# LemonATsu/UNet-PhaseGen

Hardware: AMD Instinct MI355X
Metric: spectrogram-frames/sec (train fwd+bwd) (higher is better)
Workload: dtype f32; 1 GPU; train.py full step (fwd + cos/sin/mag loss + bwd + Adam), UNetModel(1024, 2048), per-GPU batch 64 x 1024 bins x 256 frames (BASELINE configs[2]); global_batch=64, frames=256, channels=1024, parallelism=dp1, grad_allreduce_payload=fp32, adam=fused into the wgrad epilogues

## Files before the change

### unet-phasegen_amd/csrc/conv_raw_wgrad.hip

```cpp
#include "conv_common.h"

namespace {

template <int KW, int S> struct GRaw {
    static constexpr int WL = 15 * S + KW;
    static constexpr int WLP = g_wlp(KW, S);
    static constexpr int NQT = RBN / KW;
    static constexpr int TNV = NQT * KW;
    static constexpr int SUB = NQT * WLP;
    static constexpr int SUBS = (SUB + 63) / 64 * 64;
    static constexpr int NE = (SUB + NT - 1) / NT;
    static constexpr int STG = RTILE_A + 2 * SUBS;
    static constexpr int SUBP = (SUB + 255) / 256 * 256;
    static_assert(WL <= WLP, "window does not fit its slot");
};

template <int KW, int S, int BF>
__device__ __forceinline__ void g_raw_bf(const IgemmParams& p) {
    using C = GRaw<KW, S>;
    __shared__ __attribute__((aligned(16))) float lds[2 * C::STG];
    const int tid = threadIdx.x, lane = tid & 63;
    const int wv = __builtin_amdgcn_readfirstlane(tid >> 6), wm = wv >> 1, wn = wv & 1;
    const int kt = dma_kt(lane, wv);
    const rsrc_t rp = make_rsrc(p.pt, p.pt_bytes), rx = make_rsrc(p.x, p.x_bytes);
    const float slopeA = act_slope(p.act_p), slopeB = act_slope(p.act_x);
    const int pbs4 = (int)p.pt_bs * 4, xbs4 = (int)p.x_bs * 4;
    const int g = logical_wg(blockIdx.x, gridDim.x, p.whole);
    const Split sp = make_split(p.tilesM * p.tilesN, p.nslab, gridDim.x, p.whole);
    int pos = split_lo(sp, g);
    const int pos_end = split_lo(sp, g + 1);
    int slot = 0;
    while (pos < pos_end) {
        const int tile = pos / p.nslab, sb = pos - tile * p.nslab;
        const int se = min(p.nslab, sb + (pos_end - pos));
        const int m0 = (tile / p.tilesN) * RBM, n0 = (tile % p.tilesN) * C::TNV;
        const int qbase = (tile % p.tilesN) * C::NQT;

        int aoff[8];
#pragma unroll
        for (int e = 0; e < 8; ++e) {
            const int m = m0 + dma_row(lane, wv, e);
            aoff[e] = m < p.M ? m * p.LP * 4 : FAR;
        }
        constexpr bool RECOMP = KW <= 5 && BF != 0;
        int choff[RECOMP ? 1 : C::NE], vv[RECOMP ? 1 : C::NE];
        if (!RECOMP) {
#pragma unroll
            for (int e = 0; e < C::NE; ++e) {
                const int idx = tid + NT * e, ql = idx / C::WLP, v = idx - ql * C::WLP;
                choff[e] = (idx < C::SUB && qbase + ql < p.Q) ? (qbase + ql) * p.Lx * 4 : FAR;
                vv[e] = v - p.p;
            }
        }
#define GRAW_CHOFF(e) (RECOMP ? ({ int t_ = tid; asm volatile("" : "+v"(t_)); const int idx_ = t_ + NT * (e), ql_ = idx_ / C::WLP; \
                                  (idx_ < C::SUB && qbase + ql_ < p.Q) ? (qbase + ql_) * p.Lx * 4 : FAR; }) : choff[RECOMP ? 0 : (e)])
#define GRAW_VV(e) (RECOMP ? ({ int t_ = tid; asm volatile("" : "+v"(t_)); const int idx_ = t_ + NT * (e); idx_ - (idx_ / C::WLP) * C::WLP - p.p; }) \
                           : vv[RECOMP ? 0 : (e)])
        constexpr bool FASTP = BF != 2 && !(KW <= 5 && BF != 0);
        constexpr bool FASTW = FASTP && KW != 4;
        constexpr int NE16 = (C::SUB / 4 + NT - 1) / NT;
        static_assert(C::WLP % 4 == 0, "16-byte window pieces");
        int pv[FASTP ? 2 : 1], woff[FASTW ? NE16 : 1];
        if (FASTW) {
#pragma unroll
            for (int e = 0; e < NE16; ++e) {
                const int f = 4 * (tid + NT * e), ql = f / C::WLP, v0 = f - ql * C::WLP;
                woff[e] = (f < C::SUB && qbase + ql < p.Q) ? ((qbase + ql) * p.Lx + v0) * 4 : FAR;
            }
        }
        if (FASTP) {
#pragma unroll
            for (int e = 0; e < 2; ++e) {
                const int m = m0 + dma16_row(lane, wv, e);
                pv[e] = m < p.M ? (m * p.LP + dma16_kc(lane)) * 4 : FAR;
            }
        }
        int bbase[4];
#pragma unroll
        for (int jb = 0; jb < 4; ++jb) {
            const int c = wn * 128 + jb * 32 + (lane & 31), qc = c / KW;
            bbase[jb] = qc * C::WLP + (c - qc * KW) + S * 8 * (lane >> 5);
        }
        AccR acc;
#pragma unroll
        for (int i = 0; i < 2; ++i)
#pragma unroll
            for (int j = 0; j < 4; ++j)
#pragma unroll
                for (int r = 0; r < 16; ++r) acc.c[i][j][r] = 0.f;

        int gb, gi;
        { const int k0 = sb * BK; gb = k0 / p.LP; gi = k0 - gb * p.LP; }
        int kc_cur = 16;

#define GRAW_ISSUE(STAGE_PTR, K0)                                                                         \
    {   float* const As = (STAGE_PTR) + wv * 64; float* const Bw = (STAGE_PTR) + RTILE_A + wv * 64;       \
        const int k0 = (K0);                                                                              \
        const int kc = p.LP - gi;                            \
        if (FASTP && kc >= 16 && gb < p.B) {                                                              \
            const int sa = gb * pbs4 + gi * 4;                                                            \
            _Pragma("unroll") for (int e = 0; e < 2; ++e) dma16s(rp, As + wv * 192 + e * 1024, pv[FASTP ? e : 0], sa); \
        } else {                                                                                          \
          int bb, ii; divmod24(k0 + kt, p.LP, p.inv_LP, bb, ii);                                          \
          const int po = bb < p.B ? bb * pbs4 + ii * 4 : OOB;                                             \
          _Pragma("unroll") for (int e = 0; e < 8; ++e) dma4(rp, As + e * 256, aoff[e] + po); }           \
        const int w0 = S * gi - p.p;                             \
        if (FASTW && kc >= 16 && gb < p.B && w0 >= 0 && w0 + C::WLP <= p.Lx) {    \
            const int sw_ = gb * xbs4 + w0 * 4;                                                           \
            _Pragma("unroll") for (int e = 0; e < NE16; ++e)                                              \
                if (4 * (e * NT + wv * 64) < C::SUB) dma16s(rx, (STAGE_PTR) + RTILE_A + 4 * (e * NT + wv * 64), woff[FASTW ? e : 0], sw_); \
        } else {                                                                                          \
        const int sb0 = gb < p.B ? gb * xbs4 : -NEVER, sb1 = (kc < 16 && gb + 1 < p.B) ? (gb + 1) * xbs4 : -NEVER; \
        _Pragma("unroll") for (int e = 0; e < C::NE; ++e) {                                               \
            if ((e + 1) * NT <= C::SUB || e * NT + wv * 64 < C::SUB) {                                    \
                const int ps = S * gi + GRAW_VV(e);                                                       \
                dma4(rx, Bw + e * NT, ((unsigned)ps < (unsigned)p.Lx && sb0 >= 0) ? sb0 + GRAW_CHOFF(e) + ps * 4 : FAR); \
            }                                                                                             \
        }                                                                                                 \
        if (kc < 16) {                                  \
            _Pragma("unroll") for (int e = 0; e < C::NE; ++e) {                                           \
                if ((e + 1) * NT <= C::SUB || e * NT + wv * 64 < C::SUB) {                                                          \
                    const int ps = GRAW_VV(e);                                                            \
                    dma4(rx, Bw + C::SUBS + e * NT, ((unsigned)ps < (unsigned)p.Lx && sb1 >= 0) ? sb1 + GRAW_CHOFF(e) + ps * 4 : FAR); \
                }                                                                                         \
            }                                                                                             \
        }                                                                                                 \
        }                                                                                                 \
        kc_next = kc < 16 ? kc : 16;                                                                      \
        gi += BK; if (gi >= p.LP) { gi -= p.LP; ++gb; }                                                   \
    }

        PG_STAMP_DECL
        int kc_next;
        GRAW_ISSUE(lds, sb * BK)
        kc_cur = kc_next;
        __syncthreads();
        for (int sl = sb; sl < se; ++sl) {
            const int cur = (sl - sb) & 1;
            PG_STAMP(0)
#if defined(PG_G_ABL) && PG_G_ABL == 1
            kc_next = 16;
#else
            GRAW_ISSUE(lds + (cur ^ 1) * C::STG, (sl + 1) * BK)
#endif
            __builtin_amdgcn_sched_barrier(0);
            PG_STAMP(1)
            {
                const float* As = lds + cur * C::STG;
                const float* Bw = As + RTILE_A;
                const int r = lane & 31, h = lane >> 5, sw = (r >> 2) & 3;
                const float* ap = As + (wm * 64 + r) * BK;
                f32x4 a[2][2];
                float b[4][8];
                if (kc_cur >= 16) {
#pragma unroll
                    for (int i = 0; i < 2; ++i) a[i][0] = *reinterpret_cast<const f32x4*>(ap + i * 32 * BK + (((2 * h) ^ sw) << 2));
#pragma unroll
                    for (int ip = 0; ip < 4; ++ip) {
                        if (ip == 2) {
#pragma unroll
                            for (int i = 0; i < 2; ++i) a[i][1] = *reinterpret_cast<const f32x4*>(ap + i * 32 * BK + (((2 * h + 1) ^ sw) << 2));
                        }
#pragma unroll
                        for (int jb = 0; jb < 4; ++jb) { b[jb][2 * ip] = Bw[bbase[jb] + S * 2 * ip]; b[jb][2 * ip + 1] = Bw[bbase[jb] + S * (2 * ip + 1)]; }
                    }
                } else {
#pragma unroll
                    for (int c = 0; c < 2; ++c)
#pragma unroll
                        for (int i = 0; i < 2; ++i) a[i][c] = *reinterpret_cast<const f32x4*>(ap + i * 32 * BK + (((2 * h + c) ^ sw) << 2));
                    typedef const volatile __attribute__((address_space(3))) float* lds_vptr;
                    const lds_vptr Bv = (lds_vptr)Bw;
                    const int shift = C::SUBS - S * kc_cur;
#pragma unroll
                    for (int i = 0; i < 8; ++i) {
                        const int d = (8 * h + i >= kc_cur) ? shift : 0;
#pragma unroll
                        for (int jb = 0; jb < 4; ++jb) b[jb][i] = Bv[bbase[jb] + S * i + d];
                    }
                }
                if (slopeA != 1.0f) {
#pragma unroll
                    for (int i = 0; i < 2; ++i)
#pragma unroll
                        for (int c = 0; c < 2; ++c)
#pragma unroll
                            for (int v = 0; v < 4; ++v) a[i][c][v] = act_apply(a[i][c][v], slopeA);
                }
                if (slopeB != 1.0f) {
#pragma unroll
                    for (int jb = 0; jb < 4; ++jb)
#pragma unroll
                        for (int i = 0; i < 8; ++i) b[jb][i] = act_apply(b[jb][i], slopeB);
                }
                if (BF) mfma_low_2x4<BF>(a, b, acc);
                else {
#pragma unroll
                    for (int kk = 0; kk < 8; ++kk) {
#pragma unroll
                        for (int i = 0; i < 2; ++i)
#pragma unroll
                            for (int j = 0; j < 4; ++j)
                                acc.c[i][j] = __builtin_amdgcn_mfma_f32_32x32x2f32(a[i][kk >> 2][kk & 3], b[j][kk], acc.c[i][j], 0, 0, 0);
                    }
                }
            }
            __builtin_amdgcn_sched_barrier(0);
            PG_STAMP(2)
            kc_cur = kc_next;
#if defined(PG_G_ABL) && PG_G_ABL == 2
            asm volatile("s_waitcnt lgkmcnt(0)\n\ts_barrier" ::: "memory");
#else
            __syncthreads();
#endif
            PG_STAMP(3)
        }
        PG_STAMP_FLUSH
#undef GRAW_ISSUE
#undef GRAW_CHOFF
#undef GRAW_VV
        if (sb == 0 && se == p.nslab) epilogue_g<S, 2, 4>(p, acc, m0, n0, lane, wm, wn, n0 + C::TNV);
        else store_partial(p.ws, g, slot, acc, tid);
        pos += se - sb;
        slot = 1;
    }
}

template <int KW, int S, int BF>
__device__ __forceinline__ void g_ps_bf(const IgemmParams& p) {
    using C = GRaw<KW, S>;
    constexpr int STG = RTILE_A + (C::SUB + 255) / 256 * 256;
    constexpr int NE16 = (C::SUB / 4 + NT - 1) / NT;
    static_assert(C::WLP % 4 == 0 && C::WLP <= 64, "16-byte window pieces; channel 0 inside the first 64 floats");
    __shared__ __attribute__((aligned(16))) float lds[2 * STG];
    const int tid = threadIdx.x, lane = tid & 63;
    const int wv = __builtin_amdgcn_readfirstlane(tid >> 6), wm = wv >> 1, wn = wv & 1;
    const rsrc_t rp = make_rsrc(p.pt, p.pt_bytes), rx = make_rsrc(p.x, p.x_bytes);
    const float slopeA = act_slope(p.act_p), slopeB = act_slope(p.act_x);
    const int pbs4 = (int)p.pt_bs * 4, xbs4 = (int)p.x_bs * 4;
    const int cps = (p.LP + 15) >> 4;
    const int g = logical_wg(blockIdx.x, gridDim.x, p.whole);
    const Split sp = make_split(p.tilesM * p.tilesN, p.nslab, gridDim.x, p.whole);
    int pos = split_lo(sp, g);
    const int pos_end = split_lo(sp, g + 1);
    int slot = 0;
    while (pos < pos_end) {
        const int tile = pos / p.nslab, sb = pos - tile * p.nslab;
        const int se = min(p.nslab, sb + (pos_end - pos));
        const int m0 = (tile / p.tilesN) * RBM, n0 = (tile % p.tilesN) * C::TNV;
        const int qbase = (tile % p.tilesN) * C::NQT;

        int pv[2], woff[NE16];
#pragma unroll
        for (int e = 0; e < 2; ++e) {
            const int m = m0 + dma16_row(lane, wv, e);
            pv[e] = m < p.M ? (m * p.LP + dma16_kc(lane)) * 4 : FAR;
        }
#pragma unroll
        for (int e = 0; e < NE16; ++e) {
            const int f = 4 * (tid + NT * e), ql = f / C::WLP, v0 = f - ql * C::WLP;
            const int off = ((qbase + ql) * p.Lx + v0 - p.p) * 4;
            woff[e] = (f < C::SUB && qbase + ql < p.Q && off >= 0) ? off : FAR;
        }
        const bool fix0 = qbase == 0 && wv == 0;
        int f0_off, f0_v;
        { const int ql = lane / C::WLP, v = lane - ql * C::WLP; f0_off = ql < p.Q ? ql * p.Lx * 4 : FAR; f0_v = v - p.p; }
        int bbase[4], pj[4];
#pragma unroll
        for (int jb = 0; jb < 4; ++jb) {
            const int c = wn * 128 + jb * 32 + (lane & 31), qc = c / KW;
            bbase[jb] = qc * C::WLP + (c - qc * KW) + S * 8 * (lane >> 5);
            pj[jb] = (c - qc * KW) + S * 8 * (lane >> 5) - p.p;
        }
        AccR acc;
#pragma unroll
        for (int i = 0; i < 2; ++i)
#pragma unroll
            for (int j = 0; j < 4; ++j)
#pragma unroll
                for (int r = 0; r < 16; ++r) acc.c[i][j][r] = 0.f;

        int gb = sb / cps, gc = sb - gb * cps;
#define GPS_ISSUE(STAGE_PTR)                                                                              \
    {   float* const As = (STAGE_PTR) + wv * 64;                                                          \
        if (gb < p.B) {                                                                                   \
            const int gi = gc << 4;                                                                       \
            const int sa = gb * pbs4 + gi * 4;                                                            \
            _Pragma("unroll") for (int e = 0; e < 2; ++e) dma16s(rp, As + wv * 192 + e * 1024, pv[e], sa); \
            const int sw_ = gb * xbs4 + S * gi * 4;                                                       \
            _Pragma("unroll") for (int e = 0; e < NE16; ++e)                                              \
                if (4 * (e * NT + wv * 64) < C::SUB) dma16s(rx, (STAGE_PTR) + RTILE_A + 4 * (e * NT + wv * 64), woff[e], sw_); \
            if (fix0) {                                                                                   \
                const int ps = S * gi + f0_v;                                                             \
                dma4(rx, (STAGE_PTR) + RTILE_A, (unsigned)ps < (unsigned)p.Lx ? gb * xbs4 + f0_off + ps * 4 : FAR); \
            }                                                                                             \
        }                                                                                                 \
        if (++gc == cps) { gc = 0; ++gb; }                                                                \
    }
        int mb = gb, mc = gc;
        GPS_ISSUE(lds)
        __syncthreads();
        for (int sl = sb; sl < se; ++sl) {
            const int cur = (sl - sb) & 1;
            GPS_ISSUE(lds + (cur ^ 1) * STG)
            __builtin_amdgcn_sched_barrier(0);
            {
                const float* As = lds + cur * STG;
                const float* Bw = As + RTILE_A;
                const int r = lane & 31, h = lane >> 5, sw = (r >> 2) & 3;
                const float* ap = As + (wm * 64 + r) * BK;
                const int gi = mc << 4, kc = p.LP - gi;
                const int w0 = S * gi;
                f32x4 a[2][2];
                float b[4][8];
#pragma unroll
                for (int i = 0; i < 2; ++i) a[i][0] = *reinterpret_cast<const f32x4*>(ap + i * 32 * BK + (((2 * h) ^ sw) << 2));
#pragma unroll
                for (int ip = 0; ip < 4; ++ip) {
                    if (ip == 2) {
#pragma unroll
                        for (int i = 0; i < 2; ++i) a[i][1] = *reinterpret_cast<const f32x4*>(ap + i * 32 * BK + (((2 * h + 1) ^ sw) << 2));
                    }
#pragma unroll
                    for (int jb = 0; jb < 4; ++jb) { b[jb][2 * ip] = Bw[bbase[jb] + S * 2 * ip]; b[jb][2 * ip + 1] = Bw[bbase[jb] + S * (2 * ip + 1)]; }
                }
                if (kc < 16) {
#pragma unroll
                    for (int i = 0; i < 2; ++i)
#pragma unroll
                        for (int c = 0; c < 2; ++c)
#pragma unroll
                            for (int v = 0; v < 4; ++v) a[i][c][v] = (8 * h + 4 * c + v < kc) ? a[i][c][v] : 0.f;
                }
                if (w0 < p.p || w0 - p.p + C::WLP > p.Lx) {
#pragma unroll
                    for (int jb = 0; jb < 4; ++jb)
#pragma unroll
                        for (int i = 0; i < 8; ++i) b[jb][i] = (unsigned)(w0 + pj[jb] + S * i) < (unsigned)p.Lx ? b[jb][i] : 0.f;
                }
                if (slopeA != 1.0f) {
#pragma unroll
                    for (int i = 0; i < 2; ++i)
#pragma unroll
                        for (int c = 0; c < 2; ++c)
#pragma unroll
                            for (int v = 0; v < 4; ++v) a[i][c][v] = act_apply(a[i][c][v], slopeA);
                }
                if (slopeB != 1.0f) {
#pragma unroll
                    for (int jb = 0; jb < 4; ++jb)
#pragma unroll
                        for (int i = 0; i < 8; ++i) b[jb][i] = act_apply(b[jb][i], slopeB);
                }
                if (BF) mfma_low_2x4<BF>(a, b, acc);
                else {
#pragma unroll
                    for (int kk = 0; kk < 8; ++kk)
#pragma unroll
                        for (int i = 0; i < 2; ++i)
#pragma unroll
                            for (int j = 0; j < 4; ++j)
                                acc.c[i][j] = __builtin_amdgcn_mfma_f32_32x32x2f32(a[i][kk >> 2][kk & 3], b[j][kk], acc.c[i][j], 0, 0, 0);
                }
            }
            __builtin_amdgcn_sched_barrier(0);
            if (++mc == cps) { mc = 0; ++mb; }
            __syncthreads();
        }
#undef GPS_ISSUE
        (void)mb;
        if (sb == 0 && se == p.nslab) epilogue_g<S, 2, 4>(p, acc, m0, n0, lane, wm, wn, n0 + C::TNV);
        else store_partial(p.ws, g, slot, acc, tid);
        pos += se - sb;
        slot = 1;
    }
}

template <int KW, int S>
__device__ __forceinline__ void g_raw_f32(const IgemmParams& p) {
    using C = GRaw<KW, S>;
    constexpr int NP = 2 * C::SUBP / 4;
    constexpr int NE2 = (NP + NT - 1) / NT;
    constexpr int STG = RTILE_A + 2 * C::SUBP;
    static_assert(C::WLP % 4 == 0 && 2 * STG * 4 <= 64 * 1024, "16-byte window pieces; LDS budget");
    __shared__ __attribute__((aligned(16))) float lds[2 * STG];
    const int tid = threadIdx.x, lane = tid & 63;
    const int wv = __builtin_amdgcn_readfirstlane(tid >> 6), wm = wv >> 1, wn = wv & 1;
    const rsrc_t rp = make_rsrc(p.pk, p.pk_bytes), rx = make_rsrc(p.qk, p.qk_bytes);
    const int qbs4 = p.qk_bs * 4, klast4 = (p.nslab - 1) * BK * 4;
    const int g = logical_wg(blockIdx.x, gridDim.x, p.whole);
    const Split sp = make_split(p.tilesM * p.tilesN, p.nslab, gridDim.x, p.whole);
    int pos = split_lo(sp, g);
    const int pos_end = split_lo(sp, g + 1);
    int slot = 0;
    while (pos < pos_end) {
        const int tile = pos / p.nslab, sb = pos - tile * p.nslab;
        const int se = min(p.nslab, sb + (pos_end - pos));
        const int m0 = (tile / p.tilesN) * RBM, n0 = (tile % p.tilesN) * C::TNV;
        const int qbase = (tile % p.tilesN) * C::NQT;
        int pv[2], woff[NE2];
#pragma unroll
        for (int e = 0; e < 2; ++e) {
            const int m = m0 + dma16_row(lane, wv, e);
            pv[e] = m < p.M ? (m * p.Kp + dma16_kc(lane)) * 4 : FAR;
        }
#pragma unroll
        for (int e = 0; e < NE2; ++e) {
            const int pc = tid + NT * e, sub = pc >= C::SUBP / 4 ? 1 : 0, f = 4 * pc - sub * C::SUBP, ql = f / C::WLP, v0 = f - ql * C::WLP;
            woff[e] = (f < C::SUB && qbase + ql < p.Q) ? ((qbase + ql) * p.Lq + v0) * 4 : FAR;
        }
        int bbase[4];
#pragma unroll
        for (int jb = 0; jb < 4; ++jb) {
            const int c = wn * 128 + jb * 32 + (lane & 31), qc = c / KW;
            bbase[jb] = qc * C::WLP + (c - qc * KW) + S * 8 * (lane >> 5);
        }
        AccR acc;
#pragma unroll
        for (int i = 0; i < 2; ++i)
#pragma unroll
            for (int j = 0; j < 4; ++j)
#pragma unroll
                for (int r = 0; r < 16; ++r) acc.c[i][j][r] = 0.f;

        int gb, gi;
        { const int k0 = sb * BK; gb = k0 / p.LP; gi = k0 - gb * p.LP; }
        int kc_cur, kc_next;
#define GRF_ISSUE(STAGE_PTR, K0)                                                                          \
    {   const int sa = min((K0) * 4, klast4);                                                             \
        _Pragma("unroll") for (int e = 0; e < 2; ++e) dma16s(rp, (STAGE_PTR) + wv * 256 + e * 1024, pv[e], sa); \
        const int kc = p.LP - gi;                                                                         \
        const int sw0 = min(gb, p.B - 1) * qbs4 + S * gi * 4;                                             \
        const int sw1 = (kc < 16 && gb + 1 < p.B) ? (gb + 1) * qbs4 : sw0;                                \
        _Pragma("unroll") for (int e = 0; e < NE2; ++e) {                                                 \
            const int pc0 = e * NT + wv * 64;                                 \
            if ((e + 1) * NT <= NP || pc0 < NP)                                                           \
                dma16s(rx, (STAGE_PTR) + RTILE_A + 4 * pc0, woff[e], pc0 >= C::SUBP / 4 ? sw1 : sw0);     \
        }                                                                                                 \
        kc_next = kc < 16 ? kc : 16;                                                                      \
        gi += BK; if (gi >= p.LP) { gi -= p.LP; ++gb; }                                                   \
    }
        PG_STAMP_DECL
        GRF_ISSUE(lds, sb * BK)
        kc_cur = kc_next;
        __syncthreads();
        for (int sl = sb; sl < se; ++sl) {
            const int cur = (sl - sb) & 1;
            PG_STAMP(0)
#if defined(PG_G_ABL) && PG_G_ABL == 1
            kc_next = 16;
#else
            GRF_ISSUE(lds + (cur ^ 1) * STG, (sl + 1) * BK)
#endif
            __builtin_amdgcn_sched_barrier(0);
            PG_STAMP(1)
            {
                const float* As = lds + cur * STG;
                const float* Bw = As + RTILE_A;
                const int r = lane & 31, h = lane >> 5, sw = (r >> 2) & 3;
                const float* ap = As + (wm * 64 + r) * BK;
                f32x4 a[2][2];
                float b[4][8];
                if (kc_cur >= 16) {
#pragma unroll
                    for (int i = 0; i < 2; ++i) a[i][0] = *reinterpret_cast<const f32x4*>(ap + i * 32 * BK + (((2 * h) ^ sw) << 2));
#pragma unroll
                    for (int ip = 0; ip < 4; ++ip) {
                        if (ip == 2) {
#pragma unroll
                            for (int i = 0; i < 2; ++i) a[i][1] = *reinterpret_cast<const f32x4*>(ap + i * 32 * BK + (((2 * h + 1) ^ sw) << 2));
                        }
#pragma unroll
                        for (int jb = 0; jb < 4; ++jb) { b[jb][2 * ip] = Bw[bbase[jb] + S * 2 * ip]; b[jb][2 * ip + 1] = Bw[bbase[jb] + S * (2 * ip + 1)]; }
                    }
                } else {
#pragma unroll
                    for (int c = 0; c < 2; ++c)
#pragma unroll
                        for (int i = 0; i < 2; ++i) a[i][c] = *reinterpret_cast<const f32x4*>(ap + i * 32 * BK + (((2 * h + c) ^ sw) << 2));
                    typedef const volatile __attribute__((address_space(3))) float* lds_vptr;
                    const lds_vptr Bv = (lds_vptr)Bw;
                    const int shift = C::SUBP - S * kc_cur;
#pragma unroll
                    for (int i = 0; i < 8; ++i) {
                        const int d = (8 * h + i >= kc_cur) ? shift : 0;
#pragma unroll
                        for (int jb = 0; jb < 4; ++jb) b[jb][i] = Bv[bbase[jb] + S * i + d];
                    }
                }
#pragma unroll
                for (int kk = 0; kk < 8; ++kk)
#pragma unroll
                    for (int i = 0; i < 2; ++i)
#pragma unroll
                        for (int j = 0; j < 4; ++j)
                            acc.c[i][j] = __builtin_amdgcn_mfma_f32_32x32x2f32(a[i][kk >> 2][kk & 3], b[j][kk], acc.c[i][j], 0, 0, 0);
            }
            __builtin_amdgcn_sched_barrier(0);
            PG_STAMP(2)
            kc_cur = kc_next;
            __syncthreads();
            PG_STAMP(3)
        }
        PG_STAMP_FLUSH
#undef GRF_ISSUE
        if (sb == 0 && se == p.nslab) epilogue_g<S, 2, 4>(p, acc, m0, n0, lane, wm, wn, n0 + C::TNV);
        else store_partial(p.ws, g, slot, acc, tid);
        pos += se - sb;
        slot = 1;
    }
}

template <int KW, int S>
__device__ __forceinline__ void g_ps_f32(const IgemmParams& p) {
    using C = GRaw<KW, S>;
    constexpr int STG = RTILE_A + (C::SUB + 255) / 256 * 256;
    constexpr int NE16 = (C::SUB / 4 + NT - 1) / NT;
    static_assert(C::WLP % 4 == 0, "16-byte window pieces");
    __shared__ __attribute__((aligned(16))) float lds[2 * STG];
    const int tid = threadIdx.x, lane = tid & 63;
    const int wv = __builtin_amdgcn_readfirstlane(tid >> 6), wm = wv >> 1, wn = wv & 1;
    const rsrc_t rp = make_rsrc(p.pk, p.pk_bytes), rx = make_rsrc(p.qk, p.qk_bytes);
    const int pbs4 = p.M * p.Kp * 4, qbs4 = p.qk_bs * 4;
    const int cps = p.Kp >> 4;
    const int g = logical_wg(blockIdx.x, gridDim.x, p.whole);
    const Split sp = make_split(p.tilesM * p.tilesN, p.nslab, gridDim.x, p.whole);
    int pos = split_lo(sp, g);
    const int pos_end = split_lo(sp, g + 1);
    int slot = 0;
    while (pos < pos_end) {
        const int tile = pos / p.nslab, sb = pos - tile * p.nslab;
        const int se = min(p.nslab, sb + (pos_end - pos));
        const int m0 = (tile / p.tilesN) * RBM, n0 = (tile % p.tilesN) * C::TNV;
        const int qbase = (tile % p.tilesN) * C::NQT;
        int pv[2], woff[NE16];
#pragma unroll
        for (int e = 0; e < 2; ++e) {
            const int m = m0 + dma16_row(lane, wv, e);
            pv[e] = m < p.M ? (m * p.Kp + dma16_kc(lane)) * 4 : FAR;
        }
#pragma unroll
        for (int e = 0; e < NE16; ++e) {
            const int f = 4 * (tid + NT * e), ql = f / C::WLP, v0 = f - ql * C::WLP;
            woff[e] = (f < C::SUB && qbase + ql < p.Q) ? ((qbase + ql) * p.Lq + v0) * 4 : FAR;
        }
        int bbase[4];
#pragma unroll
        for (int jb = 0; jb < 4; ++jb) {
            const int c = wn * 128 + jb * 32 + (lane & 31), qc = c / KW;
            bbase[jb] = qc * C::WLP + (c - qc * KW) + S * 8 * (lane >> 5);
        }
        AccR acc;
#pragma unroll
        for (int i = 0; i < 2; ++i)
#pragma unroll
            for (int j = 0; j < 4; ++j)
#pragma unroll
                for (int r = 0; r < 16; ++r) acc.c[i][j][r] = 0.f;

        int gb = sb / cps, gc = sb - gb * cps;
#define GPF_ISSUE(STAGE_PTR)                                                                              \
    {   const int gbc = min(gb, p.B - 1), gi = gc << 4;                                                   \
        _Pragma("unroll") for (int e = 0; e < 2; ++e) dma16s(rp, (STAGE_PTR) + wv * 256 + e * 1024, pv[e], gbc * pbs4 + gi * 4); \
        const int sw_ = gbc * qbs4 + S * gi * 4;                                                          \
        _Pragma("unroll") for (int e = 0; e < NE16; ++e)                                                  \
            if (4 * (e * NT + wv * 64) < C::SUB) dma16s(rx, (STAGE_PTR) + RTILE_A + 4 * (e * NT + wv * 64), woff[e], sw_); \
        if (++gc == cps) { gc = 0; ++gb; }                                                                \
    }
        GPF_ISSUE(lds)
        __syncthreads();
        for (int sl = sb; sl < se; ++sl) {
            const int cur = (sl - sb) & 1;
            GPF_ISSUE(lds + (cur ^ 1) * STG)
            __builtin_amdgcn_sched_barrier(0);
            {
                const float* As = lds + cur * STG;
                const float* Bw = As + RTILE_A;
                const int r = lane & 31, h = lane >> 5, sw = (r >> 2) & 3;
                const float* ap = As + (wm * 64 + r) * BK;
                f32x4 a[2][2];
                float b[4][8];
#pragma unroll
                for (int i = 0; i < 2; ++i) a[i][0] = *reinterpret_cast<const f32x4*>(ap + i * 32 * BK + (((2 * h) ^ sw) << 2));
#pragma unroll
                for (int ip = 0; ip < 4; ++ip) {
                    if (ip == 2) {
#pragma unroll
                        for (int i = 0; i < 2; ++i) a[i][1] = *reinterpret_cast<const f32x4*>(ap + i * 32 * BK + (((2 * h + 1) ^ sw) << 2));
                    }
#pragma unroll
                    for (int jb = 0; jb < 4; ++jb) { b[jb][2 * ip] = Bw[bbase[jb] + S * 2 * ip]; b[jb][2 * ip + 1] = Bw[bbase[jb] + S * (2 * ip + 1)]; }
                }
#pragma unroll
                for (int kk = 0; kk < 8; ++kk)
#pragma unroll
                    for (int i = 0; i < 2; ++i)
#pragma unroll
                        for (int j = 0; j < 4; ++j)
                            acc.c[i][j] = __builtin_amdgcn_mfma_f32_32x32x2f32(a[i][kk >> 2][kk & 3], b[j][kk], acc.c[i][j], 0, 0, 0);
            }
            __builtin_amdgcn_sched_barrier(0);
            __syncthreads();
        }
#undef GPF_ISSUE
        if (sb == 0 && se == p.nslab) epilogue_g<S, 2, 4>(p, acc, m0, n0, lane, wm, wn, n0 + C::TNV);
        else store_partial(p.ws, g, slot, acc, tid);
        pos += se - sb;
        slot = 1;
    }
}

template <int KW, int S, int BF>
__global__ __launch_bounds__(NT, 2) void conv_g_raw_kernel(const IgemmParams p) {
    if constexpr (BF == 0) g_raw_f32<KW, S>(p);
    else g_raw_bf<KW, S, BF>(p);
}
template <int KW, int S, int BF>
__global__ __launch_bounds__(NT, 2) void conv_g_ps_kernel(const IgemmParams p) {
    if constexpr (BF == 0) g_ps_f32<KW, S>(p);
    else g_ps_bf<KW, S, BF>(p);
}

__global__ __launch_bounds__(256) void pack_rows_kernel(const float* __restrict__ src, long bs, int C, int L, int F, int W, unsigned n,
                                                       float slope, float* __restrict__ dst) {
    for (unsigned i = blockIdx.x * 256u + threadIdx.x; i < n; i += gridDim.x * 256u) {
        const unsigned r = i / (unsigned)W, b = r / (unsigned)C, c = r - b * (unsigned)C;
        const int t = (int)(i - r * (unsigned)W) - F;
        float v = 0.f;
        if ((unsigned)t < (unsigned)L) {
            v = src[(long)b * bs + (long)c * L + t];
            if (slope != 1.0f) v = act_apply(v, slope);
        }
        dst[i] = v;
    }
}
__global__ __launch_bounds__(256) void pack_flat_kernel(const float* __restrict__ src, long bs, int B, int LP, int Kp, unsigned n,
                                                       float slope, float* __restrict__ dst) {
    for (unsigned i = blockIdx.x * 256u + threadIdx.x; i < n; i += gridDim.x * 256u) {
        const unsigned m = i / (unsigned)Kp, k = i - m * (unsigned)Kp, b = k / (unsigned)LP, t = k - b * (unsigned)LP;
        float v = 0.f;
        if ((int)b < B) {
            v = src[(long)b * bs + (long)m * LP + t];
            if (slope != 1.0f) v = act_apply(v, slope);
        }
        dst[i] = v;
    }
}
unsigned pack_grid(unsigned n) { return (n + 255u) / 256u < 2048u ? (n + 255u) / 256u : 2048u; }

hipError_t pack_g(const IgemmParams& p, hipStream_t st) {
    float* const qk = const_cast<float*>(p.qk);
    float* const pk = const_cast<float*>(p.pk);
    const unsigned nq = (unsigned)(p.qk_bytes / 4), np = (unsigned)(p.pk_bytes / 4);
    hipLaunchKernelGGL(pack_rows_kernel, dim3(pack_grid(nq)), dim3(256), 0, st, p.x, p.x_bs, p.Q, p.Lx, p.p, p.Lq, nq, act_slope(p.act_x), qk);
    if (p.g_ps) hipLaunchKernelGGL(pack_rows_kernel, dim3(pack_grid(np)), dim3(256), 0, st, p.pt, p.pt_bs, p.M, p.LP, 0, p.Kp, np, act_slope(p.act_p), pk);
    else hipLaunchKernelGGL(pack_flat_kernel, dim3(pack_grid(np)), dim3(256), 0, st, p.pt, p.pt_bs, p.B, p.LP, p.Kp, np, act_slope(p.act_p), pk);
    return hipGetLastError();
}

template <int KW, int S>
hipError_t launch_g_raw(const IgemmParams& p, int grid, hipStream_t st, int prec) {
    if (prec == 0) {
        if (hipError_t e = pack_g(p, st)) return e;
    }
    if (p.g_ps) {
        if (prec == 1) hipLaunchKernelGGL((conv_g_ps_kernel<KW, S, 1>), dim3(grid), dim3(NT), 0, st, p);
        else if (prec == 2) hipLaunchKernelGGL((conv_g_ps_kernel<KW, S, 2>), dim3(grid), dim3(NT), 0, st, p);
        else hipLaunchKernelGGL((conv_g_ps_kernel<KW, S, 0>), dim3(grid), dim3(NT), 0, st, p);
        return hipGetLastError();
    }
    if (prec == 1) hipLaunchKernelGGL((conv_g_raw_kernel<KW, S, 1>), dim3(grid), dim3(NT), 0, st, p);
    else if (prec == 2) hipLaunchKernelGGL((conv_g_raw_kernel<KW, S, 2>), dim3(grid), dim3(NT), 0, st, p);
    else hipLaunchKernelGGL((conv_g_raw_kernel<KW, S, 0>), dim3(grid), dim3(NT), 0, st, p);
    return hipGetLastError();
}

}

hipError_t pgconv::launch_raw_g(const IgemmParams& p, int grid, hipStream_t st, int prec) {
    if (p.k == 32) return launch_g_raw<32, 2>(p, grid, st, prec);
    if (p.k == 8 && p.s == 1) return launch_g_raw<8, 1>(p, grid, st, prec);
    if (p.k == 8) return launch_g_raw<8, 2>(p, grid, st, prec);
    if (p.k == 5) return launch_g_raw<5, 2>(p, grid, st, prec);
    return launch_g_raw<4, 2>(p, grid, st, prec);
}
```

Baseline: 98760 frames/s.

## Add triple-buffered f32 wgrad pipeline and fuse vectorized pack kernels

Adds a triple-buffered f32 weight-gradient GEMM path that spreads the global-to-LDS gathers and next-slab LDS fragment reads between individual MFMA instructions, with explicit vmcnt/lgkm waits. It is meant to hide load latency behind matrix math. This path is compiled only when PG_G_PIPE is nonzero, and that macro defaults to 0. The pack kernels for Q and P are also merged into one launch that reads and writes float4 when aligned, which cuts one launch and the scalar memory traffic. The new pack path rejects shapes whose lengths are not multiples of 4, and the fused pack handles batches on a second grid axis.

New measurement: 98940 frames/s (median of 6 runs). About the same (+0.2%).

```diff
diff --git a/unet-phasegen_amd/csrc/conv_raw_wgrad.hip b/unet-phasegen_amd/csrc/conv_raw_wgrad.hip
--- a/unet-phasegen_amd/csrc/conv_raw_wgrad.hip
+++ b/unet-phasegen_amd/csrc/conv_raw_wgrad.hip
@@ -610,51 +610,328 @@
     }
 }
 
+#ifndef PG_G_PIPE
+#define PG_G_PIPE 0
+#endif
+template <int N> __device__ __forceinline__ void gw_wait_vmcnt() {
+    static_assert(N >= 0 && N < 64, "vmcnt is a 6-bit count");
+    __builtin_amdgcn_s_waitcnt((N & 15) | ((N >> 4) << 14) | (7 << 4) | (15 << 8));
+}
+__device__ __forceinline__ void gw_lgkm0() { __builtin_amdgcn_s_waitcnt(0xc07f); }
+__device__ __forceinline__ unsigned gw_lds_addr(const float* p) {
+    return (unsigned)(size_t)(const __attribute__((address_space(3))) float*)p;
+}
+struct GFrag { f32x4 a[2][2]; f32x2 b[4][4]; };
+template <int S, int N> __device__ __forceinline__ void gw_read(GFrag& f, unsigned a0, unsigned a1, const unsigned (&ba)[4]) {
+    if constexpr (N < 2) asm volatile("ds_read_b128 %0, %1 offset:%2" : "=v"(f.a[N][0]) : "v"(a0), "n"(N * 32 * BK * 4));
+    else if constexpr (N == 10 || N == 11) asm volatile("ds_read_b128 %0, %1 offset:%2" : "=v"(f.a[N - 10][1]) : "v"(a1), "n"((N - 10) * 32 * BK * 4));
+    else {
+        constexpr int q = N < 10 ? N - 2 : N - 4, ip = q >> 2, jb = q & 3;
+        asm volatile("ds_read2_b32 %0, %1 offset0:%2 offset1:%3" : "=v"(f.b[jb][ip]) : "v"(ba[jb]), "n"(S * 2 * ip), "n"(S * 2 * ip + S));
+    }
+}
+template <int S> __device__ __forceinline__ void gw_read_all(GFrag& f, unsigned a0, unsigned a1, const unsigned (&ba)[4]) {
+    gw_read<S, 0>(f, a0, a1, ba); gw_read<S, 1>(f, a0, a1, ba); gw_read<S, 2>(f, a0, a1, ba); gw_read<S, 3>(f, a0, a1, ba);
+    gw_read<S, 4>(f, a0, a1, ba); gw_read<S, 5>(f, a0, a1, ba); gw_read<S, 6>(f, a0, a1, ba); gw_read<S, 7>(f, a0, a1, ba);
+    gw_read<S, 8>(f, a0, a1, ba); gw_read<S, 9>(f, a0, a1, ba); gw_read<S, 10>(f, a0, a1, ba); gw_read<S, 11>(f, a0, a1, ba);
+    gw_read<S, 12>(f, a0, a1, ba); gw_read<S, 13>(f, a0, a1, ba); gw_read<S, 14>(f, a0, a1, ba); gw_read<S, 15>(f, a0, a1, ba);
+    gw_read<S, 16>(f, a0, a1, ba); gw_read<S, 17>(f, a0, a1, ba); gw_read<S, 18>(f, a0, a1, ba); gw_read<S, 19>(f, a0, a1, ba);
+}
+#ifndef PG_G_WAITPOS
+#define PG_G_WAITPOS 32
+#endif
+static_assert(PG_G_WAITPOS >= 10 && PG_G_WAITPOS + 20 <= 60, "gathers, barrier, reads, wait: in this order inside one slab");
+template <int S, int C, typename Issue, typename Wait>
+__device__ __forceinline__ void gw_work(GFrag& nxt, unsigned a0, unsigned a1, const unsigned (&ba)[4], const Issue& issue, const Wait& wait) {
+    if constexpr (C < 10 && (C & 1) == 0) issue(C >> 1);
+    if constexpr (C == PG_G_WAITPOS - 1) wait();
+#if PG_G_PIPE == 3
+    if constexpr (C == PG_G_WAITPOS - 1) { __builtin_amdgcn_sched_barrier(0); gw_read_all<S>(nxt, a0, a1, ba); }
+#else
+    if constexpr (C >= PG_G_WAITPOS && C < PG_G_WAITPOS + 20) gw_read<S, (C >= PG_G_WAITPOS && C < PG_G_WAITPOS + 20) ? C - PG_G_WAITPOS : 0>(nxt, a0, a1, ba);
+#endif
+    if constexpr (C == 60) gw_lgkm0();
+}
+template <int S, typename Issue, typename Wait>
+__device__ __forceinline__ void gw_slab(const GFrag& cur, GFrag& nxt, unsigned a0, unsigned a1, const unsigned (&ba)[4], AccR& acc,
+                                        const Issue& issue, const Wait& wait) {
+#define GW_CHUNK(C)                                                                                                              \
+    __builtin_amdgcn_sched_barrier(0);                                                                                           \
+    acc.c[((C) >> 2) & 1][(C) & 3] = __builtin_amdgcn_mfma_f32_32x32x2f32(cur.a[((C) >> 2) & 1][(C) >> 5][((C) >> 3) & 3],       \
+        cur.b[(C) & 3][(C) >> 4][((C) >> 3) & 1], acc.c[((C) >> 2) & 1][(C) & 3], 0, 0, 0);                                      \
+    gw_work<S, (C)>(nxt, a0, a1, ba, issue, wait);
+#define GW_ROW(C0) GW_CHUNK(C0) GW_CHUNK(C0 + 1) GW_CHUNK(C0 + 2) GW_CHUNK(C0 + 3) GW_CHUNK(C0 + 4) GW_CHUNK(C0 + 5) GW_CHUNK(C0 + 6) GW_CHUNK(C0 + 7)
+    GW_ROW(0) GW_ROW(8) GW_ROW(16) GW_ROW(24) GW_ROW(32) GW_ROW(40) GW_ROW(48) GW_ROW(56)
+    __builtin_amdgcn_sched_barrier(0);
+#undef GW_ROW
+#undef GW_CHUNK
+}
+
+template <int KW, int S, bool PS>
+__device__ __forceinline__ void g_f32_pipe(const IgemmParams& p) {
+    using C = GRaw<KW, S>;
+    constexpr int NSUB = PS ? 1 : 2;
+    constexpr int NP = NSUB * C::SUBP / 4;
+    constexpr int NE = (NP + NT - 1) / NT;
+    constexpr int STG = RTILE_A + NSUB * C::SUBP;
+    constexpr int ND = 2 + NE;
+    constexpr bool TAILALL = NE * NT <= NP;
+    static_assert(C::WLP % 4 == 0, "16-byte window pieces");
+    static_assert(3 * STG * 4 <= 64 * 1024 && 2 * 3 * STG * 4 <= 160 * 1024, "LDS budget: two workgroups per CU");
+    static_assert(ND <= 5 && NE >= 1, "gather slots of a slab");
+    __shared__ __attribute__((aligned(16))) float lds[3 * STG];
+    const int tid = threadIdx.x, lane = tid & 63;
+    const int wv = __builtin_amdgcn_readfirstlane(tid >> 6), wm = wv >> 1, wn = wv & 1;
+    const rsrc_t rp = make_rsrc(p.pk, p.pk_bytes), rx = make_rsrc(p.qk, p.qk_bytes);
+    const int qbs4 = p.qk_bs * 4, klast4 = (p.nslab - 1) * BK * 4;
+    const int pbs4 = p.M * p.Kp * 4, cps = p.Kp >> 4;
+    const bool tailw = TAILALL || (NE - 1) * NT + wv * 64 < NP;
+    const int r = lane & 31, h = lane >> 5, sw = (r >> 2) & 3;
+    const unsigned la0 = (unsigned)(((wm * 64 + r) * BK + (((2 * h) ^ sw) << 2)) * 4);
+    const unsigned la1 = (unsigned)(((wm * 64 + r) * BK + (((2 * h + 1) ^ sw) << 2)) * 4);
+    const unsigned lds0 = gw_lds_addr(lds);
+    const int g = logical_wg(blockIdx.x, gridDim.x, p.whole);
+    const Split sp = make_split(p.tilesM * p.tilesN, p.nslab, gridDim.x, p.whole);
+    int pos = split_lo(sp, g);
+    const int pos_end = split_lo(sp, g + 1);
+    int slot = 0;
+    while (pos < pos_end) {
+        const int tile = pos / p.nslab, sb = pos - tile * p.nslab;
+        const int se = min(p.nslab, sb + (pos_end - pos));
+        const int m0 = (tile / p.tilesN) * RBM, n0 = (tile % p.tilesN) * C::TNV;
+        const int qbase = (tile % p.tilesN) * C::NQT;
+        int pv[2], woff[NE];
+#pragma unroll
+        for (int e = 0; e < 2; ++e) {
+            const int m = m0 + dma16_row(lane, wv, e);
+            pv[e] = m < p.M ? (m * p.Kp + dma16_kc(lane)) * 4 : FAR;
+        }
+#pragma unroll
+        for (int e = 0; e < NE; ++e) {
+            const int pc = tid + NT * e, sub = pc >= C::SUBP / 4 ? 1 : 0, f = 4 * pc - sub * C::SUBP, ql = f / C::WLP, v0 = f - ql * C::WLP;
+            woff[e] = (f < C::SUB && qbase + ql < p.Q) ? ((qbase + ql) * p.Lq + v0) * 4 : FAR;
+        }
+        unsigned lb[4];
+#pragma unroll
+        for (int jb = 0; jb < 4; ++jb) {
+            const int c = wn * 128 + jb * 32 + (lane & 31), qc = c / KW;
+            lb[jb] = (unsigned)((RTILE_A + qc * C::WLP + (c - qc * KW) + S * 8 * (lane >> 5)) * 4);
+        }
+        AccR acc;
+#pragma unroll
+        for (int i = 0; i < 2; ++i)
+#pragma unroll
+            for (int j = 0; j < 4; ++j)
+#pragma unroll
+                for (int q = 0; q < 16; ++q) acc.c[i][j][q] = 0.f;
+
+        int gs = sb, gb, gi;
+        if (PS) { gb = sb / cps; gi = sb - gb * cps; }
+        else { const int k0 = sb * BK; gb = k0 / p.LP; gi = k0 - gb * p.LP; }
+        int sa = 0, sw0 = 0, sw1 = 0;
+        float* gstage = lds;
+        auto gather_next = [&](float* stage) __attribute__((always_inline)) {
+            gstage = stage;
+            const int gbc = min(gb, p.B - 1);
+            if (PS) {
+                sa = gbc * pbs4 + gi * 64;
+                sw0 = gbc * qbs4 + S * gi * 64;
+                if (++gi == cps) { gi = 0; ++gb; }
+            } else {
+                sa = min(gs * BK * 4, klast4);
+                sw0 = gbc * qbs4 + S * gi * 4;
+                sw1 = (p.LP - gi < 16 && gb + 1 < p.B) ? (gb + 1) * qbs4 : sw0;
+                gi += BK; if (gi >= p.LP) { gi -= p.LP; ++gb; }
+            }
+            ++gs;
+        };
+        auto issue = [&](int e) __attribute__((always_inline)) {
+            if (e < 2) dma16s(rp, gstage + wv * 256 + e * 1024, pv[e < 2 ? e : 0], sa);
+            else if (e < ND) {
+                const int x = e - 2, pc0 = x * NT + wv * 64;
+                if ((x + 1) * NT <= NP || pc0 < NP)
+                    dma16s(rx, gstage + RTILE_A + 4 * pc0, woff[x < NE ? x : 0], (!PS && pc0 >= C::SUBP / 4) ? sw1 : sw0);
+            }
+        };
+        auto wait = [&]() __attribute__((always_inline)) {
+            if (tailw) gw_wait_vmcnt<ND>(); else gw_wait_vmcnt<ND - 1>();
+            __builtin_amdgcn_s_barrier();
+            asm volatile("" ::: "memory");
+        };
+        int mi = 0;
+        if (!PS) { const int k0 = sb * BK; mi = k0 - (k0 / p.LP) * p.LP; }
+
+#pragma unroll
+        for (int hf = 0; hf < 2; ++hf) {
+            gather_next(lds + hf * STG);
+#pragma unroll
+            for (int e = 0; e < ND; ++e) issue(e);
+        }
+        __builtin_amdgcn_sched_barrier(0);
+        wait();
+        GFrag f0, f1;
+        {
+            unsigned ba[4];
+#pragma unroll
+            for (int jb = 0; jb < 4; ++jb) ba[jb] = lds0 + lb[jb];
+            gw_read_all<S>(f0, lds0 + la0, lds0 + la1, ba);
+            gw_lgkm0();
+            __builtin_amdgcn_sched_barrier(0);
+        }
+        int st = 0;
+        auto slab = [&](GFrag& cur, GFrag& nxt) __attribute__((always_inline)) {
+            const int st1 = st == 2 ? 0 : st + 1, st2 = st >= 1 ? st - 1 : 2;
+            if (!PS) {
+                const int kc = p.LP - mi;
+                if (kc < 16) {
+                    const unsigned sbase = lds0 + (unsigned)(st * STG * 4);
+                    const int shift4 = (C::SUBP - S * kc) * 4;
+                    float t[4][8];
+#pragma unroll
+                    for (int i = 0; i < 8; ++i) {
+                        const unsigned d = (8 * h + i >= kc) ? (unsigned)shift4 : 0u;
+#pragma unroll
+                        for (int jb = 0; jb < 4; ++jb)
+                            asm volatile("ds_read_b32 %0, %1 offset:%2" : "=v"(t[jb][i]) : "v"(sbase + lb[jb] + d), "n"(S * i * 4));
+                    }
+                    gw_lgkm0();
+                    __builtin_amdgcn_sched_barrier(0);
+#pragma unroll
+                    for (int jb = 0; jb < 4; ++jb)
+#pragma unroll
+                        for (int i = 0; i < 8; ++i) cur.b[jb][i >> 1][i & 1] = t[jb][i];
+                }
+                mi += BK; if (mi >= p.LP) mi -= p.LP;
+            }
+            gather_next(lds + st2 * STG);
+            const unsigned nbase = lds0 + (unsigned)(st1 * STG * 4);
+            unsigned ba[4];
+#pragma unroll
+            for (int jb = 0; jb < 4; ++jb) ba[jb] = nbase + lb[jb];
+            gw_slab<S>(cur, nxt, nbase + la0, nbase + la1, ba, acc, issue, wait);
+            st = st1;
+        };
+        for (int sl = sb;;) {
+            slab(f0, f1);
+            if (++sl >= se) break;
+            slab(f1, f0);
+            if (++sl >= se) break;
+        }
+        __syncthreads();
+        if (sb == 0 && se == p.nslab) epilogue_g<S, 2, 4>(p, acc, m0, n0, lane, wm, wn, n0 + C::TNV);
+        else store_partial(p.ws, g, slot, acc, tid);
+        pos += se - sb;
+        slot = 1;
+    }
+}
+
+template <int KW, int S> constexpr bool g_pipe_fits(bool ps) { return 3 * (RTILE_A + (ps ? 1 : 2) * GRaw<KW, S>::SUBP) * 4 <= 64 * 1024; }
+
 template <int KW, int S, int BF>
 __global__ __launch_bounds__(NT, 2) void conv_g_raw_kernel(const IgemmParams p) {
-    if constexpr (BF == 0) g_raw_f32<KW, S>(p);
-    else g_raw_bf<KW, S, BF>(p);
+    if constexpr (BF != 0) g_raw_bf<KW, S, BF>(p);
+    else if constexpr (PG_G_PIPE != 0 && g_pipe_fits<KW, S>(false)) g_f32_pipe<KW, S, false>(p);
+    else g_raw_f32<KW, S>(p);
 }
 template <int KW, int S, int BF>
 __global__ __launch_bounds__(NT, 2) void conv_g_ps_kernel(const IgemmParams p) {
-    if constexpr (BF == 0) g_ps_f32<KW, S>(p);
-    else g_ps_bf<KW, S, BF>(p);
-}
-
-__global__ __launch_bounds__(256) void pack_rows_kernel(const float* __restrict__ src, long bs, int C, int L, int F, int W, unsigned n,
-                                                       float slope, float* __restrict__ dst) {
-    for (unsigned i = blockIdx.x * 256u + threadIdx.x; i < n; i += gridDim.x * 256u) {
-        const unsigned r = i / (unsigned)W, b = r / (unsigned)C, c = r - b * (unsigned)C;
-        const int t = (int)(i - r * (unsigned)W) - F;
-        float v = 0.f;
-        if ((unsigned)t < (unsigned)L) {
-            v = src[(long)b * bs + (long)c * L + t];
-            if (slope != 1.0f) v = act_apply(v, slope);
-        }
-        dst[i] = v;
-    }
-}
-__global__ __launch_bounds__(256) void pack_flat_kernel(const float* __restrict__ src, long bs, int B, int LP, int Kp, unsigned n,
-                                                       float slope, float* __restrict__ dst) {
-    for (unsigned i = blockIdx.x * 256u + threadIdx.x; i < n; i += gridDim.x * 256u) {
-        const unsigned m = i / (unsigned)Kp, k = i - m * (unsigned)Kp, b = k / (unsigned)LP, t = k - b * (unsigned)LP;
-        float v = 0.f;
-        if ((int)b < B) {
-            v = src[(long)b * bs + (long)m * LP + t];
-            if (slope != 1.0f) v = act_apply(v, slope);
-        }
-        dst[i] = v;
-    }
-}
-unsigned pack_grid(unsigned n) { return (n + 255u) / 256u < 2048u ? (n + 255u) / 256u : 2048u; }
+    if constexpr (BF != 0) g_ps_bf<KW, S, BF>(p);
+    else if constexpr (PG_G_PIPE != 0 && g_pipe_fits<KW, S>(true)) g_f32_pipe<KW, S, true>(p);
+    else g_ps_f32<KW, S>(p);
+}
+
+struct PackOp {
+    const float* src; float* dst; long bs;
+    int flat, B, C, L, F, W;
+    float inv_L;
+    int div, dst16;
+    float slope;
+};
+__device__ __forceinline__ void pack_store(float* d, const f32x4& v, int dst16) {
+    if (dst16) *reinterpret_cast<f32x4*>(d) = v;
+    else { d[0] = v[0]; d[1] = v[1]; d[2] = v[2]; d[3] = v[3]; }
+}
+__global__ __launch_bounds__(256) void pack_g_kernel(const PackOp oq, const PackOp op) {
+    const PackOp& o = blockIdx.z ? op : oq;
+    const unsigned W4 = (unsigned)o.W >> 2;
+    if (!o.flat) {
+        const unsigned n = (unsigned)o.C * W4;
+        for (int b = blockIdx.y; b < o.B; b += gridDim.y) {
+            const float* sb_ = o.src + (long)b * o.bs;
+            float* db = o.dst + (long)b * o.C * o.W;
+            for (unsigned i = blockIdx.x * 256u + threadIdx.x; i < n; i += gridDim.x * 256u) {
+                const unsigned c = i / W4;
+                const int t0 = (int)(4u * (i - c * W4)) - o.F;
+                const float* s = sb_ + (long)c * o.L + t0;
+                f32x4 v = {0.f, 0.f, 0.f, 0.f};
+                if (t0 >= 0 && t0 + 4 <= o.L && ((uintptr_t)s & 15) == 0) v = *reinterpret_cast<const f32x4*>(s);
+                else {
+#pragma unroll
+                    for (int e = 0; e < 4; ++e)
+                        if ((unsigned)(t0 + e) < (unsigned)o.L) v[e] = s[e];
+                }
+                if (o.slope != 1.0f) {
+#pragma unroll
+                    for (int e = 0; e < 4; ++e) v[e] = act_apply(v[e], o.slope);
+                }
+                pack_store(db + 4l * i, v, o.dst16);
+            }
+        }
+    } else {
+        const unsigned n = (unsigned)o.C * W4;
+        const unsigned nb = gridDim.x * gridDim.y;
+        for (unsigned i = (blockIdx.y * gridDim.x + blockIdx.x) * 256u + threadIdx.x; i < n; i += nb * 256u) {
+            const unsigned m = i / W4;
+            const int k0 = (int)(4u * (i - m * W4));
+            int b, t;
+            if (o.div) { b = k0 / o.L; t = k0 - b * o.L; }
+            else divmod24(k0, o.L, o.inv_L, b, t);
+            const float* s = o.src + (long)b * o.bs + (long)m * o.L + t;
+            f32x4 v = {0.f, 0.f, 0.f, 0.f};
+            if (b < o.B && t + 4 <= o.L && ((uintptr_t)s & 15) == 0) v = *reinterpret_cast<const f32x4*>(s);
+            else {
+#pragma unroll
+                for (int e = 0; e < 4; ++e) {
+                    if (b < o.B) v[e] = o.src[(long)b * o.bs + (long)m * o.L + t];
+                    if (++t == o.L) { t = 0; ++b; }
+                }
+            }
+            if (o.slope != 1.0f) {
+#pragma unroll
+                for (int e = 0; e < 4; ++e) v[e] = act_apply(v[e], o.slope);
+            }
+            pack_store(o.dst + 4l * i, v, o.dst16);
+        }
+    }
+}
+PackOp pack_rows_op(const float* src, long bs, int B, int C, int L, int F, int W, float slope, float* dst) {
+    PackOp o{};
+    o.src = src; o.dst = dst; o.bs = bs; o.flat = 0; o.B = B; o.C = C; o.L = L; o.F = F; o.W = W; o.slope = slope;
+    o.dst16 = ((uintptr_t)dst & 15) == 0;
+    return o;
+}
+PackOp pack_flat_op(const float* src, long bs, int B, int M, int LP, int Kp, float slope, float* dst) {
+    PackOp o{};
+    o.src = src; o.dst = dst; o.bs = bs; o.flat = 1; o.B = B; o.C = M; o.L = LP; o.F = 0; o.W = Kp; o.slope = slope;
+    o.inv_L = 1.0f / (float)LP; o.div = Kp >= (1 << 24);
+    o.dst16 = ((uintptr_t)dst & 15) == 0;
+    return o;
+}
 
 hipError_t pack_g(const IgemmParams& p, hipStream_t st) {
-    float* const qk = const_cast<float*>(p.qk);
-    float* const pk = const_cast<float*>(p.pk);
-    const unsigned nq = (unsigned)(p.qk_bytes / 4), np = (unsigned)(p.pk_bytes / 4);
-    hipLaunchKernelGGL(pack_rows_kernel, dim3(pack_grid(nq)), dim3(256), 0, st, p.x, p.x_bs, p.Q, p.Lx, p.p, p.Lq, nq, act_slope(p.act_x), qk);
-    if (p.g_ps) hipLaunchKernelGGL(pack_rows_kernel, dim3(pack_grid(np)), dim3(256), 0, st, p.pt, p.pt_bs, p.M, p.LP, 0, p.Kp, np, act_slope(p.act_p), pk);
-    else hipLaunchKernelGGL(pack_flat_kernel, dim3(pack_grid(np)), dim3(256), 0, st, p.pt, p.pt_bs, p.B, p.LP, p.Kp, np, act_slope(p.act_p), pk);
+    if ((p.Lq & 3) || (p.Kp & 3)) return hipErrorInvalidValue;
+    const PackOp oq = pack_rows_op(p.x, p.x_bs, p.B, p.Q, p.Lx, p.p, p.Lq, act_slope(p.act_x), const_cast<float*>(p.qk));
+    const PackOp op = p.g_ps ? pack_rows_op(p.pt, p.pt_bs, p.B, p.M, p.LP, 0, p.Kp, act_slope(p.act_p), const_cast<float*>(p.pk))
+                             : pack_flat_op(p.pt, p.pt_bs, p.B, p.M, p.LP, p.Kp, act_slope(p.act_p), const_cast<float*>(p.pk));
+    const unsigned gy = (unsigned)(p.B < 64 ? p.B : 64);
+    const auto blocks = [gy](const PackOp& o) {
+        const unsigned long n = (unsigned long)o.C * (unsigned)(o.W >> 2);
+        return (unsigned)(((o.flat ? (n + gy - 1) / gy : n) + 255) / 256);
+    };
+    unsigned gx = blocks(oq) > blocks(op) ? blocks(oq) : blocks(op);
+    const unsigned cap = 4096u / gy;
+    gx = gx < 1u ? 1u : (gx > cap ? cap : gx);
+    hipLaunchKernelGGL(pack_g_kernel, dim3(gx, gy, 2), dim3(256), 0, st, oq, op);
     return hipGetLastError();
 }
 
```
